# bbuhrow/avx-ecm

Hardware: AMD Instinct MI355X
Metric: stage-1 curves/sec at B1=1000000, 416-bit N (higher is better)
Workload: dtype u32 (28-bit limbs, 64-bit accumulate)

## Files before the change

avx-ecm_amd/csrc/gecm_row.hpp:

```cpp
#pragma once
#include "gecm_curve.hpp"
#include "gecm_rowk.h"

template <int NQ>
struct FeR {
    int32_t v[NQ];
};

template <int NQ>
struct RowMod {
    uint32_t n[NQ];
    uint32_t rho;
    int32_t c16;
    int32_t kb, zb;
};

__device__ __forceinline__ void row_pin(const int64_t &x)
{
    asm volatile("" ::"v"(x));
}
__device__ __forceinline__ int32_t row_c16()
{
    int32_t c;
    asm volatile("s_mov_b32 %0, 16" : "=s"(c));
    return c;
}
template <int32_t V>
__device__ __forceinline__ int32_t row_bias()
{
    int32_t c;
    asm volatile("v_mov_b32 %0, %1" : "=v"(c) : "n"(V));
    return c;
}

#define GECM_DPP_ROW_SHL1 0x101
#define GECM_DPP_ROW_SHR1 0x111
#define GECM_DPP_ROW_ROR1 0x121
#define GECM_DPP_ROW_NEWBCAST 0x150

template <int CTRL>
__device__ __forceinline__ uint32_t row_dpp(uint32_t x)
{
    return (uint32_t)__builtin_amdgcn_update_dpp(0, (int)x, CTRL, 0xF, 0xF, true);
}
template <int I>
__device__ __forceinline__ uint32_t row_bcast(uint32_t x)
{
    return row_dpp<GECM_DPP_ROW_NEWBCAST + I>(x);
}
template <int I>
__device__ __forceinline__ int64_t row_bcast64(int64_t x)
{
    return __builtin_amdgcn_update_dpp((int64_t)0, x, GECM_DPP_ROW_NEWBCAST + I, 0xF, 0xF, true);
}
template <int I>
__device__ __forceinline__ uint32_t row_bcast_lds(uint32_t x)
{
    return (uint32_t)__builtin_amdgcn_ds_swizzle((int)x, 0x10 | (I << 5));
}
__device__ __forceinline__ uint32_t other_row(uint32_t x)
{
    return (uint32_t)__builtin_amdgcn_ds_swizzle((int)x, 0x401F );
}

__device__ __forceinline__ void smad(int64_t &acc, int32_t x, int32_t y)
{
    asm("v_mad_i64_i32 %0, vcc, %1, %2, %0" : "+v"(acc) : "v"(x), "v"(y) : "vcc");
}
__device__ __forceinline__ void umad(int64_t &acc, uint32_t x, uint32_t y)
{
    asm("v_mad_u64_u32 %0, vcc, %1, %2, %0" : "+v"(acc) : "v"(x), "v"(y) : "vcc");
}
__device__ __forceinline__ int64_t smad0(int32_t x, int32_t y)
{
    int64_t r;
    asm("v_mad_i64_i32 %0, vcc, %1, %2, 0" : "=v"(r) : "v"(x), "v"(y) : "vcc");
    return r;
}
__device__ __forceinline__ int64_t smad16(int32_t x, int64_t add)
{
    int64_t r;
    asm("v_mad_i64_i32 %0, vcc, %1, 16, %2" : "=v"(r) : "v"(x), "v"(add) : "vcc");
    return r;
}

__device__ __forceinline__ int64_t smad16_smad(int32_t x, int64_t add, int32_t y, int32_t z)
{
    int64_t r;
    asm("v_mad_i64_i32 %0, vcc, %1, 16, %2\n\tv_mad_i64_i32 %0, vcc, %3, %4, %0" : "=&v"(r) : "v"(x), "v"(add), "v"(y), "v"(z) : "vcc");
    return r;
}

template <int NQ, int ROWS, bool RHO1, bool ALDS, bool A4 = false, bool B4 = false, bool R4 = false>
__device__ __forceinline__ void fer_mul(FeR<NQ> &r, const FeR<NQ> &a, const FeR<NQ> &b, const RowMod<NQ> &m)
{
    static_assert(ROWS > 16 * (NQ - 1) && ROWS <= 16 * NQ, "the limbs in use fill the lanes but for the last one");
    static_assert(!ALDS || NQ == 1, "the crossbar form is for one limb per lane");
    int32_t a4[NQ], b4[NQ];
#pragma unroll
    for (int t = 0; t < NQ; t++) {
        a4[t] = A4 ? a.v[t] : (int32_t)((uint32_t)a.v[t] << 2);
        b4[t] = B4 ? b.v[t] : (int32_t)((uint32_t)b.v[t] << 2);
    }
    if constexpr (NQ >= 2) {
        int64_t T[NQ];
        const int64_t a01 = (int64_t)(((uint64_t)(uint32_t)a4[1] << 32) | (uint32_t)a4[0]);
        int64_t Ap = row_bcast64<0>(a01);
        int32_t As = 0;
        auto limb = [&](auto jc) -> int32_t {
            constexpr int q = decltype(jc)::value % NQ;
            return q == 0 ? (int32_t)(uint32_t)Ap : q == 1 ? (int32_t)(Ap >> 32) : As;
        };
#pragma unroll
        for (int t = 0; t < NQ; t++) T[t] = (int64_t)limb(IC<0>{}) * b4[t];
        static_for<0, ROWS>([&](auto ic) {
            constexpr int i = decltype(ic)::value;
            constexpr int rot = i % NQ, nxt = (i + 1) % NQ;
            const uint32_t Q = row_bcast<0>(RHO1 ? (uint32_t)T[rot] : (uint32_t)T[rot] * m.rho);
            __builtin_amdgcn_sched_barrier(0);
#pragma unroll
            for (int t = 0; t < NQ; t++) {
                T[(t + rot) % NQ] = (int64_t)((uint64_t)T[(t + rot) % NQ] + (uint64_t)Q * m.n[t]);
                __builtin_amdgcn_sched_barrier(0);
            }
            const int32_t Ac = limb(IC<i + 1>{});
            if constexpr (i + 1 < ROWS) {
#pragma unroll
                for (int t = 0; t < NQ - 1; t++) {
                    T[(t + nxt) % NQ] += (int64_t)Ac * b4[t];
                    row_pin(T[(t + nxt) % NQ]);
                    __builtin_amdgcn_sched_barrier(0);
                }
            }
            const int32_t hi = (int32_t)(T[rot] >> 32);
            const uint32_t lo = row_dpp<GECM_DPP_ROW_SHL1>((uint32_t)T[rot]);
            __builtin_amdgcn_sched_barrier(0);
            T[nxt] += (int64_t)hi * m.c16;
            row_pin(T[nxt]);
            __builtin_amdgcn_sched_barrier(0);
            if constexpr (i + 1 < ROWS) {
                T[rot] = (int64_t)Ac * b4[NQ - 1] + (int64_t)(uint64_t)lo;
                row_pin(T[rot]);
            } else {
                T[rot] = (int64_t)(uint64_t)lo;
            }
            __builtin_amdgcn_sched_barrier(0);
            if constexpr (i + 2 < ROWS) {
                if constexpr ((i + 2) % NQ == 0) Ap = row_bcast64<(i + 2) / NQ>(a01);
                else if constexpr ((i + 2) % NQ == 2) As = (int32_t)row_bcast<(i + 2) / NQ>((uint32_t)a4[NQ - 1]);
                __builtin_amdgcn_sched_barrier(0);
            }
        });
        int32_t lo[NQ];
        int32_t carry = 0;
#pragma unroll
        for (int t = 0; t < NQ - 1; t++) {
            int64_t u16 = T[(t + ROWS) % NQ] + (int64_t)(1u << 31);
            if (t > 0) u16 += (int64_t)carry * m.c16;
            carry = (int32_t)(u16 >> 32);
            lo[t] = (int32_t)(((uint32_t)u16 >> 4) & GECM_LIMB_MASK) - (1 << 27);
        }
        const int32_t ut = (int32_t)(T[(NQ - 1 + ROWS) % NQ] >> 4) + carry + (1 << 27);
        lo[NQ - 1] = (int32_t)((uint32_t)ut & GECM_LIMB_MASK) - (1 << 27);
        const int32_t below = (int32_t)row_dpp<GECM_DPP_ROW_SHR1>((uint32_t)(ut >> GECM_LIMB_BITS));
        lo[0] += below;
#pragma unroll
        for (int t = 0; t < NQ; t++) r.v[t] = R4 ? (int32_t)((uint32_t)lo[t] << 2) : lo[t];
    } else {
        int32_t Ab[ROWS];
        int64_t a01 = 0;
        if constexpr (!ALDS) a01 = (int64_t)(((uint64_t)row_dpp<GECM_DPP_ROW_SHL1>((uint32_t)a4[0]) << 32) | (uint32_t)a4[0]);
        auto request = [&](auto jc) {
            constexpr int j = decltype(jc)::value;
            if constexpr (ALDS) {
                Ab[j] = (int32_t)row_bcast_lds<j>((uint32_t)a4[0]);
            } else if constexpr (j % 2 == 0) {
                const int64_t P = row_bcast64<j>(a01);
                Ab[j] = (int32_t)(uint32_t)P;
                if constexpr (j + 1 < ROWS) Ab[j + 1] = (int32_t)(P >> 32);
            }
        };
        if constexpr (ALDS) static_for<0, ROWS>(request);
        else request(IC<0>{});
        int64_t T[NQ];
#pragma unroll
        for (int t = 0; t < NQ; t++) T[t] = 0;
        static_for<0, ROWS>([&](auto ic) {
            constexpr int i = decltype(ic)::value;
            if constexpr (i == 0) T[0] = smad0(Ab[0], b4[0]);
            if constexpr (!ALDS) {
                __builtin_amdgcn_sched_barrier(0);
                if constexpr (i + 1 < ROWS) request(IC<i + 1>{});
                __builtin_amdgcn_sched_barrier(0);
            }
            uint32_t qs = (uint32_t)T[0];
            if (!RHO1) qs *= m.rho;
            const uint32_t Q = row_bcast<0>(qs);
            umad(T[0], Q, m.n[0]);
            if constexpr (!ALDS) __builtin_amdgcn_sched_barrier(0);
            const int32_t hi = (int32_t)(T[0] >> 32);
            const uint32_t lo = row_dpp<GECM_DPP_ROW_SHL1>((uint32_t)T[0]);
            int64_t add = (int64_t)(uint64_t)lo;
            if constexpr (R4 && i + 2 == ROWS) add = (int64_t)(((uint64_t)(uint32_t)m.kb << 32) | lo);
            if constexpr (R4 && i + 1 == ROWS) add = (int64_t)(((uint64_t)(uint32_t)m.zb << 32) | lo);
            if constexpr (i + 1 < ROWS) T[0] = smad16_smad(hi, add, Ab[i + 1], b4[0]);
            else T[0] = smad16(hi, add);
        });
        if constexpr (R4) {
            r.v[0] = (int32_t)(((uint32_t)T[0] >> 2) + (row_dpp<GECM_DPP_ROW_ROR1>((uint32_t)(T[0] >> 32)) << 2));
        } else {
            const int64_t u16 = T[0] + (int64_t)(1u << 31);
            const int32_t lim = (int32_t)(((uint32_t)u16 >> 4) & GECM_LIMB_MASK) - (1 << 27);
            r.v[0] = lim + (int32_t)row_dpp<GECM_DPP_ROW_SHR1>((uint32_t)(u16 >> 32));
        }
    }
}

template <int NQ>
struct PtR {
    FeR<NQ> own;
    FeR<NQ> oth;
};

struct RowSign {
    uint32_t mz, bz;
    uint32_t mx, bx;
};

template <int NQ>
__device__ __forceinline__ void fer_other(FeR<NQ> &r, const FeR<NQ> &a)
{
#pragma unroll
    for (int t = 0; t < NQ; t++) r.v[t] = (int32_t)other_row((uint32_t)a.v[t]);
}

template <int NQ>
__device__ __forceinline__ void fer_sum_diff(FeR<NQ> &r, const FeR<NQ> &oth, const FeR<NQ> &own, const RowSign &g)
{
#pragma unroll
    for (int t = 0; t < NQ; t++) r.v[t] = (int32_t)((uint32_t)oth.v[t] + ((uint32_t)own.v[t] ^ g.mz) + g.bz);
}

template <int NQ>
__device__ __forceinline__ void row_sd(FeR<NQ> &r, const PtR<NQ> &p, const RowSign &g)
{
    fer_sum_diff<NQ>(r, p.oth, p.own, g);
}

template <int NQ>
__device__ __forceinline__ void row_ds(FeR<NQ> &r, const PtR<NQ> &p, const RowSign &g)
{
#pragma unroll
    for (int t = 0; t < NQ; t++) r.v[t] = (int32_t)((uint32_t)p.own.v[t] + ((uint32_t)p.oth.v[t] ^ g.mx) + g.bx);
}

template <int NQ>
__device__ __forceinline__ void row_pick(FeR<NQ> &r, const FeR<NQ> &a, const FeR<NQ> &b, uint64_t pick)
{
#pragma unroll
    for (int t = 0; t < NQ; t++) {
        int32_t x;
        asm volatile("v_cndmask_b32 %0, %1, %2, %3" : "=v"(x) : "v"(a.v[t]), "v"(b.v[t]), "s"(pick));
        r.v[t] = x;
    }
}

template <int NQ, int ROWS, bool ALDS>
__device__ __forceinline__ void row_add(FeR<NQ> &own, const FeR<NQ> &fB, const FeR<NQ> &fA, const FeR<NQ> &c, bool isZ,
                                        const RowSign &g, const RowMod<NQ> &m)
{
    FeR<NQ> w, t, e;
    fer_mul<NQ, ROWS, true, ALDS, true, true, true>(w, fB, fA, m);
    fer_other<NQ>(t, w);
    fer_sum_diff<NQ>(e, t, w, g);
    fer_mul<NQ, ROWS, true, ALDS, true, true, true>(e, e, e, m);
    fer_mul<NQ, ROWS, true, ALDS, true, true, true>(own, e, c, m);
}

template <int NQ, int ROWS, bool ALDS>
__device__ __forceinline__ void row_dup(FeR<NQ> &own, const FeR<NQ> &fA, const FeR<NQ> &s4, bool isZ, const RowSign &g,
                                        const RowMod<NQ> &m)
{
    FeR<NQ> q, t, w, p1, p2, r1;
    fer_mul<NQ, ROWS, true, ALDS, true, true, true>(q, fA, fA, m);
    fer_other<NQ>(t, q);
#pragma unroll
    for (int i = 0; i < NQ; i++) {
        w.v[i] = t.v[i] - q.v[i];
        p1.v[i] = isZ ? s4.v[i] : q.v[i];
        p2.v[i] = isZ ? w.v[i] : t.v[i];
    }
    fer_mul<NQ, ROWS, true, ALDS, true, true, true>(r1, p1, p2, m);
#pragma unroll
    for (int i = 0; i < NQ; i++) t.v[i] = r1.v[i] + q.v[i];
    fer_mul<NQ, ROWS, true, ALDS, true, true, true>(t, t, w, m);
#pragma unroll
    for (int i = 0; i < NQ; i++) own.v[i] = isZ ? t.v[i] : r1.v[i];
}

template <int NQ>
__device__ __forceinline__ void fer_load(FeR<NQ> &r, const uint32_t *__restrict__ base, size_t stride, uint32_t cidx,
                                         uint32_t l, uint32_t nl)
{
#pragma unroll
    for (int t = 0; t < NQ; t++) {
        const uint32_t limb = (uint32_t)NQ * l + (uint32_t)t;
        r.v[t] = limb < nl ? (int32_t)base[(size_t)limb * stride + cidx] : 0;
    }
}

template <int NQ, int ROWS, bool ALDS>
__device__ __forceinline__ void run_tape_row(const uint32_t *__restrict__ tape, uint32_t tape_len, PtR<NQ> &A,
                                             const FeR<NQ> &s4, bool isZ, const RowSign &g, const RowMod<NQ> &m)
{
    PtR<NQ> B = A;
    FeR<NQ> Coth = A.oth;
    auto fetch = [&](uint32_t pc) -> uint32_t {
        uint32_t w = tape[pc >> 2];
        return __builtin_amdgcn_readfirstlane((w >> ((pc & 3u) * 8u)) & 0xffu);
    };
    uint32_t nxt = tape_len ? fetch(0) : GECM_OP_NOP;
    for (uint32_t pc = 0; pc < tape_len; pc++) {
        uint32_t op = nxt;
        nxt = (pc + 1 < tape_len) ? fetch(pc + 1) : GECM_OP_NOP;
        while ((op & ~GECM_OP_SWAP) == (GECM_OP_STEP | GECM_OP_RULE3)) {
            const uint64_t swap = (op & GECM_OP_SWAP) ? ~(uint64_t)0 : 0;
            FeR<NQ> fA, fB;
            row_sd<NQ>(fA, A, g);
            row_ds<NQ>(fB, B, g);
            row_pick<NQ>(A.own, A.own, B.own, swap);
            row_add<NQ, ROWS, ALDS>(B.own, fB, fA, Coth, isZ, g, m);
            row_pick<NQ>(Coth, B.oth, A.oth, swap);
            row_pick<NQ>(A.oth, A.oth, B.oth, swap);
            fer_other<NQ>(B.oth, B.own);
            pc++;
            op = nxt;
            nxt = (pc + 1 < tape_len) ? fetch(pc + 1) : GECM_OP_NOP;
        }
        if (op == GECM_OP_NOP) continue;
        const uint32_t rule = op & GECM_OP_RULE_MASK;
        const bool is_step = op >= GECM_OP_STEP;
        const bool do_add = op != GECM_OP_PRAC_BEGIN;
        const bool do_dup = op != GECM_OP_PRAC_END;
        PtR<NQ> C;
        C.oth = Coth;
        fer_other<NQ>(C.own, Coth);
        if (is_step && (op & GECM_OP_SWAP)) {
            PtR<NQ> t = A;
            A = B;
            B = t;
        }
        if (is_step && rule == GECM_OP_RULE5) {
            PtR<NQ> t = B;
            B = C;
            C = t;
        } else if (is_step && rule == GECM_OP_RULE9) {
            PtR<NQ> t = A;
            A = B;
            B = C;
            C = t;
        } else if (op == GECM_OP_PRAC_BEGIN) {
            B = A;
            C = A;
        }
        PtR<NQ> T, D;
        FeR<NQ> fA, fB;
        row_sd<NQ>(fA, A, g);
        row_ds<NQ>(fB, B, g);
        if (do_add) {
            row_add<NQ, ROWS, ALDS>(T.own, fB, fA, C.oth, isZ, g, m);
            fer_other<NQ>(T.oth, T.own);
        }
        if (do_dup) {
            row_dup<NQ, ROWS, ALDS>(D.own, fA, s4, isZ, g, m);
            fer_other<NQ>(D.oth, D.own);
        }
        if (op == GECM_OP_PRAC_END) {
            A = T;
        } else if (op == GECM_OP_PRAC_BEGIN) {
            A = D;
        } else if (rule == GECM_OP_RULE4) {
            B = T;
            A = D;
        } else if (rule == GECM_OP_RULE5) {
            PtR<NQ> t = C;
            C = T;
            B = t;
            A = D;
        } else {
            PtR<NQ> oldA = C;
            C = T;
            B = D;
            A = oldA;
        }
        Coth = C.oth;
    }
}


template <int NQ, int ROWS, bool ALDS>
__device__ __forceinline__ void stage1_row(const uint32_t *__restrict__ tape, uint32_t tape_len, uint32_t *__restrict__ X,
                                           uint32_t *__restrict__ Z, const uint32_t *__restrict__ S, size_t stride,
                                           uint32_t nl, const uint32_t *__restrict__ rc, uint32_t rho_n)
{
    const uint32_t cidx = (blockIdx.x * blockDim.x + threadIdx.x) >> 5;
    const uint32_t l = threadIdx.x & 15u;
    const bool isZ = (threadIdx.x & 16u) != 0;
    uint32_t *mine = isZ ? Z : X;
    RowMod<NQ> mp, mn;
    FeR<NQ> cin, one, kp;
#pragma unroll
    for (int t = 0; t < NQ; t++) {
        const uint32_t j = (uint32_t)NQ * l + (uint32_t)t;
        mp.n[t] = rc[0 * GECM_ROW_WORDS + j];
        mn.n[t] = rc[1 * GECM_ROW_WORDS + j];
        cin.v[t] = (int32_t)rc[2 * GECM_ROW_WORDS + j];
        one.v[t] = (int32_t)rc[3 * GECM_ROW_WORDS + j];
        kp.v[t] = (int32_t)rc[4 * GECM_ROW_WORDS + j];
    }
    mp.rho = 1u;
    mn.rho = rho_n;
    mp.c16 = mn.c16 = row_c16();
    mp.kb = mn.kb = mp.zb = mn.zb = 0;
    if constexpr (NQ == 1) {
        mp.kb = mn.kb = row_bias<(1 << 27)>();
        mp.zb = mn.zb = row_bias<-(1 << 27)>();
    }
    PtR<NQ> P;
    FeR<NQ> s4, t;
    fer_load<NQ>(t, mine, stride, cidx, l, nl);
    fer_mul<NQ, ROWS, true, ALDS, false, false, true>(P.own, t, cin, mp);
    RowSign g;
    g.mz = isZ ? 0xffffffffu : 0u;
    g.bz = isZ ? 1u : 0u;
    g.mx = ~g.mz;
    g.bx = 1u - g.bz;
    fer_other<NQ>(P.oth, P.own);
    fer_load<NQ>(t, S, stride, cidx, l, nl);
    fer_mul<NQ, ROWS, true, ALDS, false, false, true>(s4, t, cin, mp);
    run_tape_row<NQ, ROWS, ALDS>(tape, tape_len, P, s4, isZ, g, mp);
    fer_mul<NQ, ROWS, false, ALDS, true>(t, P.own, one, mn);
    uint32_t u[NQ];
#pragma unroll
    for (int i = 0; i < NQ; i++) u[i] = (uint32_t)(t.v[i] + kp.v[i]);
    const uint32_t below = row_dpp<GECM_DPP_ROW_SHR1>(u[NQ - 1] >> GECM_LIMB_BITS);
#pragma unroll
    for (int i = 0; i < NQ; i++) {
        const uint32_t limb = (uint32_t)NQ * l + (uint32_t)i;
        const uint32_t v = (u[i] & GECM_LIMB_MASK) + (i == 0 ? below : (u[i - 1] >> GECM_LIMB_BITS));
        if (limb < nl) mine[(size_t)limb * stride + cidx] = (limb == nl - 1) ? v + (u[i] & ~GECM_LIMB_MASK) : v;
    }
}


template <int NQ, int ROWS>
__device__ __forceinline__ void fer_reduce(FeR<NQ> &v, const RowMod<NQ> &m, float minv, uint32_t l)
{
    constexpr int TL = (ROWS - 1) / NQ, TS = (ROWS - 1) % NQ;
    const int32_t top = (int32_t)row_bcast<TL>((uint32_t)v.v[TS]);
    const int32_t q = (int32_t)__builtin_rintf((float)top * minv);
    int32_t lo[NQ], c[NQ];
#pragma unroll
    for (int t = 0; t < NQ; t++) {
        const int32_t x = v.v[t] - q * (int32_t)m.n[t];
        const bool split = (uint32_t)NQ * l + (uint32_t)t < (uint32_t)(ROWS - 1);
        c[t] = split ? (x + (1 << 27)) >> GECM_LIMB_BITS : 0;
        lo[t] = x - (int32_t)((uint32_t)c[t] << GECM_LIMB_BITS);
    }
    v.v[0] = lo[0] + (int32_t)row_dpp<GECM_DPP_ROW_SHR1>((uint32_t)c[NQ - 1]);
#pragma unroll
    for (int t = 1; t < NQ; t++) v.v[t] = lo[t] + c[t - 1];
}

template <int NQ>
struct UnitRow {
    RowMod<NQ> m;
    FeR<NQ> two;
    float minv;
    uint32_t l;
    bool pp1;
};

template <int NQ, int ROWS>
__device__ __forceinline__ void unit_row_add(FeR<NQ> &T, const FeR<NQ> &X, const FeR<NQ> &Y, const FeR<NQ> &W,
                                             const UnitRow<NQ> &u)
{
    fer_mul<NQ, ROWS, true, false>(T, X, Y, u.m);
    if (u.pp1) {
#pragma unroll
        for (int t = 0; t < NQ; t++) T.v[t] -= W.v[t];
        fer_reduce<NQ, ROWS>(T, u.m, u.minv, u.l);
    }
}

template <int NQ, int ROWS>
__device__ __forceinline__ void run_tape_unit_row(const uint32_t *__restrict__ tape, uint32_t tape_len, FeR<NQ> &A,
                                                  const UnitRow<NQ> &u)
{
    FeR<NQ> B = A, C = A;
    auto fetch = [&](uint32_t pc) -> uint32_t {
        uint32_t w = tape[pc >> 2];
        return __builtin_amdgcn_readfirstlane((w >> ((pc & 3u) * 8u)) & 0xffu);
    };
    uint32_t nxt = tape_len ? fetch(0) : GECM_OP_NOP;
    for (uint32_t pc = 0; pc < tape_len; pc++) {
        uint32_t op = nxt;
        nxt = (pc + 1 < tape_len) ? fetch(pc + 1) : GECM_OP_NOP;
        while ((op & ~GECM_OP_SWAP) == (GECM_OP_STEP | GECM_OP_RULE3)) {
            if (op & GECM_OP_SWAP) {
                FeR<NQ> t = A;
                A = B;
                B = t;
            }
            FeR<NQ> T;
            unit_row_add<NQ, ROWS>(T, B, A, C, u);
            C = B;
            B = T;
            pc++;
            op = nxt;
            nxt = (pc + 1 < tape_len) ? fetch(pc + 1) : GECM_OP_NOP;
        }
        if (op == GECM_OP_NOP) continue;
        const uint32_t rule = op & GECM_OP_RULE_MASK;
        const bool is_step = op >= GECM_OP_STEP;
        const bool do_add = op != GECM_OP_PRAC_BEGIN;
        const bool do_dup = op != GECM_OP_PRAC_END;
        if (is_step && (op & GECM_OP_SWAP)) {
            FeR<NQ> t = A;
            A = B;
            B = t;
        }
        if (is_step && rule == GECM_OP_RULE5) {
            FeR<NQ> t = B;
            B = C;
            C = t;
        } else if (is_step && rule == GECM_OP_RULE9) {
            FeR<NQ> t = A;
            A = B;
            B = C;
            C = t;
        } else if (op == GECM_OP_PRAC_BEGIN) {
            B = A;
            C = A;
        }
        FeR<NQ> T, D;
        if (do_add) unit_row_add<NQ, ROWS>(T, B, A, C, u);
        if (do_dup) unit_row_add<NQ, ROWS>(D, A, A, u.two, u);
        if (op == GECM_OP_PRAC_END) {
            A = T;
        } else if (op == GECM_OP_PRAC_BEGIN) {
            A = D;
        } else if (rule == GECM_OP_RULE4) {
            B = T;
            A = D;
        } else if (rule == GECM_OP_RULE5) {
            FeR<NQ> t = C;
            C = T;
            B = t;
            A = D;
        } else {
            FeR<NQ> oldA = C;
            C = T;
            B = D;
            A = oldA;
        }
    }
}

template <int NQ, int ROWS>
__device__ __forceinline__ void unit_row(const uint32_t *__restrict__ tape, uint32_t tape_len, uint32_t *__restrict__ X,
                                         size_t stride, uint32_t nl, bool pp1, const uint32_t *__restrict__ rc)
{
    const uint32_t pos = (blockIdx.x * blockDim.x + threadIdx.x) >> 4;
    const uint32_t l = threadIdx.x & 15u;
    UnitRow<NQ> u;
    RowMod<NQ> mn;
    FeR<NQ> cin, one, kp;
#pragma unroll
    for (int t = 0; t < NQ; t++) {
        const uint32_t j = (uint32_t)NQ * l + (uint32_t)t;
        u.m.n[t] = rc[0 * GECM_ROW_WORDS + j];
        mn.n[t] = rc[1 * GECM_ROW_WORDS + j];
        cin.v[t] = (int32_t)rc[2 * GECM_ROW_WORDS + j];
        one.v[t] = (int32_t)rc[3 * GECM_ROW_WORDS + j];
        kp.v[t] = (int32_t)rc[4 * GECM_ROW_WORDS + j];
        u.two.v[t] = (int32_t)rc[5 * GECM_ROW_WORDS + j];
    }
    u.minv = __uint_as_float(rc[6 * GECM_ROW_WORDS + 0]);
    u.m.rho = 1u;
    mn.rho = rc[6 * GECM_ROW_WORDS + 1];
    u.m.c16 = mn.c16 = row_c16();
    u.l = l;
    u.pp1 = pp1;
    FeR<NQ> A, t;
    fer_load<NQ>(t, X, stride, pos, l, nl);
    fer_mul<NQ, ROWS, true, false>(A, t, cin, u.m);
    fer_reduce<NQ, ROWS>(A, u.m, u.minv, l);
    run_tape_unit_row<NQ, ROWS>(tape, tape_len, A, u);
    fer_mul<NQ, ROWS, false, false>(t, A, one, mn);
    uint32_t w[NQ];
#pragma unroll
    for (int i = 0; i < NQ; i++) w[i] = (uint32_t)(t.v[i] + kp.v[i]);
    const uint32_t below = row_dpp<GECM_DPP_ROW_SHR1>(w[NQ - 1] >> GECM_LIMB_BITS);
#pragma unroll
    for (int i = 0; i < NQ; i++) {
        const uint32_t limb = (uint32_t)NQ * l + (uint32_t)i;
        const uint32_t v = (w[i] & GECM_LIMB_MASK) + (i == 0 ? below : (w[i - 1] >> GECM_LIMB_BITS));
        if (limb < nl) X[(size_t)limb * stride + pos] = (limb == nl - 1) ? v + (w[i] & ~GECM_LIMB_MASK) : v;
    }
}
```

Baseline: 1686.

## Precompute row broadcasts of add operands ahead of the multiply chain

Adds a RowScan that gathers all DPP row broadcasts of one multiplicand up front, and a scanned fer_mul variant that consumes them instead of interleaving broadcasts with the multiply-accumulate chain. In the differential add, the broadcasts of fA and of the C coordinate are issued early, and the swap picks and tape fetch are interleaved between multiplies to fill latency. This removes DPP broadcast latency from the critical path of the serial MAD chain, at the cost of holding ROWS extra registers per scan, which may raise register pressure and lower occupancy.

Result: faster. 1707 (median of 6 runs) (+1.2%).

```diff
diff --git a/avx-ecm_amd/csrc/gecm_row.hpp b/avx-ecm_amd/csrc/gecm_row.hpp
--- a/avx-ecm_amd/csrc/gecm_row.hpp
+++ b/avx-ecm_amd/csrc/gecm_row.hpp
@@ -91,11 +91,18 @@
     return r;
 }
 
-template <int NQ, int ROWS, bool RHO1, bool ALDS, bool A4 = false, bool B4 = false, bool R4 = false>
-__device__ __forceinline__ void fer_mul(FeR<NQ> &r, const FeR<NQ> &a, const FeR<NQ> &b, const RowMod<NQ> &m)
+template <int ROWS>
+struct RowScan {
+    int32_t Ab[ROWS];
+};
+
+template <int NQ, int ROWS, bool RHO1, bool ALDS, bool A4 = false, bool B4 = false, bool R4 = false, bool SCANNED = false>
+__device__ __forceinline__ void fer_mul(FeR<NQ> &r, const FeR<NQ> &a, const FeR<NQ> &b, const RowMod<NQ> &m,
+                                        const RowScan<ROWS> *scan = nullptr)
 {
     static_assert(ROWS > 16 * (NQ - 1) && ROWS <= 16 * NQ, "the limbs in use fill the lanes but for the last one");
     static_assert(!ALDS || NQ == 1, "the crossbar form is for one limb per lane");
+    static_assert(!SCANNED || (NQ == 1 && !ALDS), "a ready-made scan is for the one-limb DPP form");
     int32_t a4[NQ], b4[NQ];
 #pragma unroll
     for (int t = 0; t < NQ; t++) {
@@ -169,10 +176,15 @@
     } else {
         int32_t Ab[ROWS];
         int64_t a01 = 0;
-        if constexpr (!ALDS) a01 = (int64_t)(((uint64_t)row_dpp<GECM_DPP_ROW_SHL1>((uint32_t)a4[0]) << 32) | (uint32_t)a4[0]);
+        if constexpr (SCANNED) {
+#pragma unroll
+            for (int j = 0; j < ROWS; j++) Ab[j] = scan->Ab[j];
+        }
+        if constexpr (!ALDS && !SCANNED) a01 = (int64_t)(((uint64_t)row_dpp<GECM_DPP_ROW_SHL1>((uint32_t)a4[0]) << 32) | (uint32_t)a4[0]);
         auto request = [&](auto jc) {
             constexpr int j = decltype(jc)::value;
-            if constexpr (ALDS) {
+            if constexpr (SCANNED) {
+            } else if constexpr (ALDS) {
                 Ab[j] = (int32_t)row_bcast_lds<j>((uint32_t)a4[0]);
             } else if constexpr (j % 2 == 0) {
                 const int64_t P = row_bcast64<j>(a01);
@@ -216,6 +228,24 @@
     }
 }
 
+template <int ROWS>
+__device__ __forceinline__ void fer_scan(RowScan<ROWS> &s, const FeR<1> &a)
+{
+    const int64_t a01 = (int64_t)(((uint64_t)row_dpp<GECM_DPP_ROW_SHL1>((uint32_t)a.v[0]) << 32) | (uint32_t)a.v[0]);
+    static_for<0, (ROWS + 1) / 2>([&](auto kc) {
+        constexpr int j = 2 * decltype(kc)::value;
+        const int64_t P = row_bcast64<j>(a01);
+        s.Ab[j] = (int32_t)(uint32_t)P;
+        if constexpr (j + 1 < ROWS) s.Ab[j + 1] = (int32_t)(P >> 32);
+    });
+    __builtin_amdgcn_sched_barrier(0);
+}
+template <int ROWS>
+__device__ __forceinline__ void fer_mul_scanned(FeR<1> &r, const RowScan<ROWS> &s, const FeR<1> &b, const RowMod<1> &m)
+{
+    fer_mul<1, ROWS, true, false, true, true, true, true>(r, b, b, m, &s);
+}
+
 template <int NQ>
 struct PtR {
     FeR<NQ> own;
@@ -275,6 +305,22 @@
     fer_sum_diff<NQ>(e, t, w, g);
     fer_mul<NQ, ROWS, true, ALDS, true, true, true>(e, e, e, m);
     fer_mul<NQ, ROWS, true, ALDS, true, true, true>(own, e, c, m);
+}
+
+template <int ROWS, class Shadow>
+__device__ __forceinline__ void row_add_scanned(FeR<1> &own, const RowScan<ROWS> &sA, const FeR<1> &fB, const FeR<1> &c,
+                                                const RowSign &g, const RowMod<1> &m, Shadow &&shadow)
+{
+    FeR<1> w, t, e;
+    RowScan<ROWS> sC;
+    fer_mul_scanned<ROWS>(w, sA, fB, m);
+    fer_other<1>(t, w);
+    fer_scan<ROWS>(sC, c);
+    shadow();
+    __builtin_amdgcn_sched_barrier(0);
+    fer_sum_diff<1>(e, t, w, g);
+    fer_mul<1, ROWS, true, false, true, true, true>(e, e, e, m);
+    fer_mul_scanned<ROWS>(own, sC, e, m);
 }
 
 template <int NQ, int ROWS, bool ALDS>
@@ -326,16 +372,33 @@
         while ((op & ~GECM_OP_SWAP) == (GECM_OP_STEP | GECM_OP_RULE3)) {
             const uint64_t swap = (op & GECM_OP_SWAP) ? ~(uint64_t)0 : 0;
             FeR<NQ> fA, fB;
-            row_sd<NQ>(fA, A, g);
-            row_ds<NQ>(fB, B, g);
-            row_pick<NQ>(A.own, A.own, B.own, swap);
-            row_add<NQ, ROWS, ALDS>(B.own, fB, fA, Coth, isZ, g, m);
-            row_pick<NQ>(Coth, B.oth, A.oth, swap);
-            row_pick<NQ>(A.oth, A.oth, B.oth, swap);
-            fer_other<NQ>(B.oth, B.own);
-            pc++;
-            op = nxt;
-            nxt = (pc + 1 < tape_len) ? fetch(pc + 1) : GECM_OP_NOP;
+            if constexpr (NQ == 1 && !ALDS) {
+                RowScan<ROWS> sA;
+                row_sd<NQ>(fA, A, g);
+                row_pick<NQ>(A.own, A.own, B.own, swap);
+                fer_scan<ROWS>(sA, fA);
+                row_ds<NQ>(fB, B, g);
+                row_add_scanned<ROWS>(B.own, sA, fB, Coth, g, m, [&]() {
+                    row_pick<NQ>(Coth, B.oth, A.oth, swap);
+                    row_pick<NQ>(A.oth, A.oth, B.oth, swap);
+                });
+                pc++;
+                op = nxt;
+                nxt = (pc + 1 < tape_len) ? fetch(pc + 1) : GECM_OP_NOP;
+                __builtin_amdgcn_sched_barrier(0);
+                fer_other<NQ>(B.oth, B.own);
+            } else {
+                row_sd<NQ>(fA, A, g);
+                row_ds<NQ>(fB, B, g);
+                row_pick<NQ>(A.own, A.own, B.own, swap);
+                row_add<NQ, ROWS, ALDS>(B.own, fB, fA, Coth, isZ, g, m);
+                row_pick<NQ>(Coth, B.oth, A.oth, swap);
+                row_pick<NQ>(A.oth, A.oth, B.oth, swap);
+                fer_other<NQ>(B.oth, B.own);
+                pc++;
+                op = nxt;
+                nxt = (pc + 1 < tape_len) ? fetch(pc + 1) : GECM_OP_NOP;
+            }
         }
         if (op == GECM_OP_NOP) continue;
         const uint32_t rule = op & GECM_OP_RULE_MASK;
@@ -368,7 +431,13 @@
         row_sd<NQ>(fA, A, g);
         row_ds<NQ>(fB, B, g);
         if (do_add) {
-            row_add<NQ, ROWS, ALDS>(T.own, fB, fA, C.oth, isZ, g, m);
+            if constexpr (NQ == 1 && !ALDS) {
+                RowScan<ROWS> sA;
+                fer_scan<ROWS>(sA, fA);
+                row_add_scanned<ROWS>(T.own, sA, fB, C.oth, g, m, []() {});
+            } else {
+                row_add<NQ, ROWS, ALDS>(T.own, fB, fA, C.oth, isZ, g, m);
+            }
             fer_other<NQ>(T.oth, T.own);
         }
         if (do_dup) {
```
